# nudro/TFC-GAN

Measured on AMD Instinct MI355X. Metric: training images/sec at 256x256 PATCH-16, 1/2/4/8 MI355X; gen L1 vs ref, higher is better.
Workload: dtype bf16; 1 GPU; PATCH-16 256x256 bf16, batch 32 per GPU (BASELINE.json configs[1]; configs[3] at 8 GPUs): G step + D step, 16-patch triplet + patch-FFT loss, Adam (step as BASELINE.md section 3 defines it: LPIPS and the temperature head excluded); global_batch=32, per_gpu_batch=32, parallelism=dp1

## Files before the change

### tfc-gan_amd/_lib.py

```python
import ctypes
import os
import subprocess
import threading

_HERE = os.path.dirname(os.path.abspath(__file__))
_ROOT = os.path.dirname(_HERE)
CSRC = os.path.join(_HERE, "csrc")
SO_PATH = os.path.join(_HERE, "libtfcgan_hip.so")
SOURCES = ["api.hip", "igemm.hip", "elementwise.hip", "losses.hip", "stn.hip", "lpips.hip", "input.hip", "probe.hip", "vit.hip"]
HEADERS = ["common.h", "tfc_desc.h", "pack_math.h"]
PUBLIC_HEADER = os.path.join(_ROOT, "include", "tfc_gan.h")

DT_BF16, DT_F32 = 0, 1
OP_CONV, OP_PADCONV, OP_CONVT, OP_UPCONV, OP_CONV3 = 0, 1, 2, 3, 4
EP_BIAS, EP_STATS, EP_ACCUM, EP_TANH_NCHW, EP_LEAKY, EP_RELU = 1, 2, 4, 8, 16, 32

_lock = threading.Lock()
_lib = None


def _stale():
    if not os.path.exists(SO_PATH):
        return True
    t = os.path.getmtime(SO_PATH)
    deps = [os.path.join(CSRC, f) for f in SOURCES + HEADERS] + [PUBLIC_HEADER]
    return any(os.path.exists(d) and os.path.getmtime(d) > t for d in deps)


def build(force=False, verbose=False):
    if not force and not _stale():
        return SO_PATH
    import fcntl
    try:
        lk = open(SO_PATH + ".lock", "w")
    except OSError:
        return _build_locked(verbose)
    with lk:
        fcntl.flock(lk, fcntl.LOCK_EX)
        try:
            if not force and not _stale():
                return SO_PATH
            return _build_locked(verbose)
        finally:
            fcntl.flock(lk, fcntl.LOCK_UN)


def _build_locked(verbose):
    hipcc = os.environ.get("HIPCC", "/opt/rocm/bin/hipcc")
    if not os.path.exists(hipcc):
        hipcc = "hipcc"
    cmd = [hipcc, "--offload-arch=gfx950", "-O3", "-std=c++17", "-fPIC", "-shared", "-Wno-unused-value", "-Rpass-analysis=kernel-resource-usage",
           "-Wl,-rpath,/opt/rocm/lib", "-o", SO_PATH + ".tmp"] + [os.path.join(CSRC, f) for f in SOURCES]
    if verbose:
        print(" ".join(cmd))
    res = subprocess.run(cmd, stderr=subprocess.PIPE, text=True)
    if res.returncode != 0:
        raise RuntimeError("hipcc failed:\n" + "\n".join(l for l in res.stderr.splitlines() if "remark:" not in l)[-8000:])
    bad = check_no_spills(res.stderr)
    if bad:
        raise RuntimeError("hand-scheduled kernels must not spill (their asm loads carry hand-counted waits the compiler cannot see): " + "; ".join(bad))
    os.replace(SO_PATH + ".tmp", SO_PATH)
    return SO_PATH


GUARDED_KERNELS = ("tfc_igemm2_kernel", "tfc_wgrad")


def check_no_spills(remarks):
    bad, name = [], None
    for line in remarks.splitlines():
        if "Function Name:" in line:
            name = line.split("Function Name:")[1].split("[")[0].strip()
        elif name and any(g in name for g in GUARDED_KERNELS):
            for key in ("ScratchSize [bytes/lane]:", "VGPRs Spill:"):
                if key in line:
                    val = int(line.split(key)[1].split("[")[0].strip())
                    if val != 0:
                        bad.append(f"{name[:80]}: {key} {val}")
    return bad


_c = ctypes
_vp, _i, _f, _ll, _u32, _sz = _c.c_void_p, _c.c_int, _c.c_float, _c.c_longlong, _c.c_uint32, _c.c_size_t

PROTOTYPES = {
    "tfc_last_error": (_c.c_char_p, []),
    "tfc_abi_version": (_i, []),
    "tfc_part_ws_floats": (_sz, []),
    "tfc_conv_packed_bytes": (_sz, [_i, _i, _i, _i, _i]),
    "tfc_conv_pack": (_i, [_vp, _i, _i, _i, _vp, _vp, _vp, _i, _i]),
    "tfc_pack_plan_bytes": (_sz, [_i]),
    "tfc_pack_plan_build": (_i, [_i, _i, _c.POINTER(_i), _c.POINTER(_i), _c.POINTER(_vp), _c.POINTER(_vp), _c.POINTER(_i), _c.POINTER(_i),
                                 _vp, _c.POINTER(_i)]),
    "tfc_conv_pack_planned": (_i, [_vp, _i, _vp, _i, _i]),
    "tfc_conv_fwd": (_i, [_vp, _i, _i, _vp, _i, _i, _i, _i, _i, _i, _vp, _vp, _i, _vp, _vp, _vp, _vp, _i, _vp]),
    "tfc_conv_dgrad_image": (_i, [_vp, _i, _vp, _i, _i, _i, _i, _i, _i, _vp, _vp, _i, _vp]),
    "tfc_upconv_head_fwd": (_i, [_vp, _i, _vp, _i, _i, _i, _i, _i, _i, _vp, _vp, _vp]),
    "tfc_upconv_head_dgrad": (_i, [_vp, _i, _vp, _i, _i, _i, _i, _i, _i, _vp, _vp, _i]),
    "tfc_patchgan_head_fwd": (_i, [_vp, _i, _vp, _i, _i, _i, _i, _i, _vp, _vp, _i]),
    "tfc_conv_dgrad": (_i, [_vp, _i, _i, _vp, _i, _i, _i, _i, _i, _i, _vp, _vp, _i, _vp, _i]),
    "tfc_conv_wgrad_ws_bytes": (_sz, [_i, _i, _i]),
    "tfc_conv_wgrad": (_i, [_vp, _i, _i, _vp, _i, _vp, _i, _i, _i, _i, _i, _i, _vp, _vp, _i]),
    "tfc_act_fwd": (_i, [_vp, _i, _vp, _i, _i, _i, _i, _i, _vp, _i, _f, _i, _f, _u32, _vp, _i, _vp, _vp]),
    "tfc_act_bwd_signs": (_i, [_vp, _i, _vp, _i, _vp, _i, _i, _i, _i, _f, _vp, _vp, _i, _vp]),
    "tfc_act_bwd": (_i, [_vp, _i, _i, _vp, _i, _vp, _i, _i, _i, _i, _i, _vp, _i, _f, _i, _f, _u32, _vp, _vp, _i, _vp]),
    "tfc_dropout_mask": (_i, [_vp, _vp, _ll, _f, _u32]),
    "tfc_pack_nhwc8": (_i, [_vp, _i, _vp, _i, _vp, _i, _vp, _i, _i, _i]),
    "tfc_unpack_nchw": (_i, [_vp, _i, _vp, _i, _i, _i, _vp, _i, _i, _i, _f, _f]),
    "tfc_tanh_bwd_pack": (_i, [_vp, _i, _vp, _vp, _vp, _vp, _i, _i, _i, _i, _vp]),
    "tfc_colsum": (_i, [_vp, _i, _vp, _ll, _i, _i, _vp, _vp]),
    "tfc_cast": (_i, [_vp, _i, _i, _vp, _vp, _ll]),
    "tfc_axpby": (_i, [_vp, _vp, _vp, _vp, _ll, _f, _f]),
    "tfc_spectral_norm_step": (_i, [_vp, _vp, _vp, _vp, _vp, _vp, _i, _i, _i]),
    "tfc_spectral_norm_batched_ws_floats": (_sz, [_i, _c.POINTER(_i), _c.POINTER(_i)]),
    "tfc_spectral_norm_step_batched": (_i, [_vp, _i, _c.POINTER(_vp), _c.POINTER(_vp), _c.POINTER(_vp), _c.POINTER(_vp), _c.POINTER(_vp),
                                            _c.POINTER(_vp), _c.POINTER(_i), _c.POINTER(_i), _vp, _i]),
    "tfc_spectral_norm_bwd": (_i, [_vp, _vp, _vp, _vp, _vp, _vp, _vp, _vp, _i, _i, _i]),
    "tfc_patch16_triplet": (_i, [_vp, _vp, _vp, _c.POINTER(_i), _i, _i, _vp, _vp, _f]),
    "tfc_fft_spectrum": (_i, [_vp, _vp, _ll, _ll, _i, _i, _i, _i, _i, _i, _vp, _vp, _i, _vp]),
    "tfc_fft_spectrum_ws_bytes": (_sz, [_i, _i]),
    "tfc_logmag_mse": (_i, [_vp, _vp, _vp, _i, _i, _vp]),
    "tfc_logmag_mae": (_i, [_vp, _vp, _vp, _i, _i, _vp]),
    "tfc_vectorize_temps": (_i, [_vp, _vp, _ll, _i, _i, _i, _i, _vp, _vp]),
    "tfc_row_triplet": (_i, [_vp, _vp, _vp, _vp, _ll, _i, _f, _vp]),
    "tfc_l1_sum": (_i, [_vp, _vp, _vp, _ll, _f, _vp, _i]),
    "tfc_affine_warp_fwd": (_i, [_vp, _vp, _vp, _vp, _i, _i, _i, _i]),
    "tfc_affine_warp_bwd": (_i, [_vp, _vp, _vp, _vp, _vp, _vp, _i, _i, _i, _i, _vp]),
    "tfc_morph_grad_fwd": (_i, [_vp, _vp, _vp, _vp, _ll, _i, _i]),
    "tfc_morph_grad_bwd": (_i, [_vp, _vp, _vp, _vp, _ll, _i, _i]),
    "tfc_row_triplet_grad": (_i, [_vp, _vp, _vp, _vp, _ll, _i, _f, _f, _vp, _vp]),
    "tfc_first_block_bwd_supported": (_i, [_i, _i, _i]),
    "tfc_first_block_bwd_wgrad": (_i, [_vp, _i, _vp, _i, _vp, _i, _vp, _i, _i, _i, _i, _i, _i, _f, _vp, _vp, _i, _vp, _vp, _vp]),
    "tfc_conv_first_fwd": (_i, [_vp, _i, _vp, _i, _i, _i, _i, _i, _i, _vp, _vp, _i, _vp, _vp, _i, _vp]),
    "tfc_first_block_fwd": (_i, [_vp, _i, _vp, _i, _i, _i, _i, _i, _i, _vp, _vp, _vp, _f, _i, _vp, _i, _vp]),
    "tfc_resize_plan_bytes": (_sz, [_i, _i, _i]),
    "tfc_resize_plan_build": (_i, [_i, _i, _i, _vp]),
    "tfc_pair_resize_ws_bytes": (_sz, [_i, _i, _i]),
    "tfc_pair_resize_normalize": (_i, [_vp, _vp, _ll, _i, _i, _vp, _vp, _vp, _vp, _vp, _vp, _vp, _vp, _vp]),
    "tfc_lpips_input_fwd": (_i, [_vp, _i, _vp, _vp, _vp, _vp, _i, _i, _i, _i, _i]),
    "tfc_lpips_input_bwd": (_i, [_vp, _i, _vp, _vp, _vp, _i, _i, _i, _i, _i, _f, _i]),
    "tfc_maxpool2_fwd": (_i, [_vp, _i, _vp, _vp, _i, _i, _i, _i]),
    "tfc_maxpool2_bwd": (_i, [_vp, _i, _vp, _vp, _vp, _i, _i, _i, _i]),
    "tfc_relu_bwd": (_i, [_vp, _i, _vp, _vp, _vp, _vp, _ll]),
    "tfc_lpips_head": (_i, [_vp, _i, _vp, _vp, _vp, _vp, _vp, _i, _i, _i, _i, _f]),
    "tfc_bce_relativistic": (_i, [_vp, _i, _vp, _vp, _i, _i, _f, _f, _i, _vp, _vp, _vp, _f]),
    "tfc_adam_step": (_i, [_vp, _vp, _vp, _vp, _vp, _ll, _f, _f, _f, _f, _i, _f]),
    "tfc_prof_enable": (_i, [_i]),
    "tfc_prof_collect": (_i, [_i, _c.POINTER(_c.c_double), _c.POINTER(_c.c_double), _c.POINTER(_ll)]),
# ... 42 lines not shown
```

### tfc-gan_amd/csrc/api.hip

```cpp
#include <hip/hip_runtime.h>
#include <math.h>
#include <stdarg.h>
#include <stdio.h>
#include <string.h>
#include <stdlib.h>
#include <string>
#include <vector>
#include "../../include/tfc_gan.h"
#undef TFC_DT_BF16
#undef TFC_DT_F32
#undef TFC_EP_BIAS
#undef TFC_EP_STATS
#undef TFC_EP_ACCUM
#undef TFC_EP_TANH_NCHW
#undef TFC_EP_LEAKY
#undef TFC_EP_RELU
#undef TFC_OP_CONV
#undef TFC_OP_PADCONV
#undef TFC_OP_CONVT
#undef TFC_OP_UPCONV
#undef TFC_OP_CONV3
#include "tfc_desc.h"
#include "pack_math.h"
#define TFC_OP_CONV 0
#define TFC_OP_PADCONV 1
#define TFC_OP_CONVT 2
#define TFC_OP_UPCONV 3
#define TFC_OP_CONV3 4

int tfc_total_substeps(const TfcGather& d, int es);
int tfc_nb32(int nout);
int tfc_nb32_padded(int nout);
size_t tfc_packed_bytes(const TfcGather& d, int es);
hipError_t tfc_launch_pack(int dt, const TfcGather& d, const float* w, const float* scale, void* wp, int Nreal, int Creal, long long sn, long long sc, hipStream_t st);
hipError_t tfc_launch_igemm(int dt, const TfcGather& d, const void* in, const void* wp, void* out, const float* bias, float* stats, float* part_ws, float* out_nchw, const float* oscale, int flags, hipStream_t st);
hipError_t tfc_launch_first_block_fwd(const void* in, int N, int IH, int IW, const void* wp, const float* bias, const float* oscale, float slope, int gform,
                                      void* out, int o_pitch, unsigned char* sign_mask, hipStream_t st);
bool tfc_conv_c8_eligible(const TfcGather& d, int flags);
hipError_t tfc_launch_conv_c8(const TfcGather& d, const void* in, const void* wp, void* out, const float* bias, const float* oscale, int flags,
                              unsigned char* sign_mask, hipStream_t st);
hipError_t tfc_launch_wgrad(int dt, const TfcGather& d, const void* dO, const void* in, float* dwacc, void* slab, int Nn_pad, int Nn_real, int Cw_real, hipStream_t st, TfcWgradFin* fin);
hipError_t tfc_launch_dgrad_rows4(const void* dy, int dy_pitch, int N, int H, int W, const float* w, int Cin, const float* oscale, int NC, float* dx, hipStream_t st);
hipError_t tfc_launch_upconv_head(const void* x, int x_pitch, int N, int H, int W, const float* w, const float* bias, int Cout, float* out, hipStream_t st);
bool tfc_launch_wgrad_phases_fused(int up, const void* x, int N, int IH, int IW, int x_pitch, int Cin_pad, const void* dy, int dy_pitch, int Cout,
                                   int Cin, float* dwacc, void* slab, hipStream_t st, hipError_t* err, TfcWgradFin* fin);
hipError_t tfc_launch_wgrad_finish(float* acc, float* grad, int Nn, int Cw, long long sn, long long sc, int accumulate, hipStream_t st);
hipError_t tfc_launch_pack_planned(int dt, const void* plan_dev, int njobs, int nblocks, hipStream_t st);
hipError_t tfc_launch_act_fwd(int dt, const ActParams& p, const void* x, const float* stats, void* out, float* stats_out, float* part_ws, hipStream_t st);
hipError_t tfc_launch_act_bwd(int dt, int mode, const ActParams& p, const void* dout, const void* x, const float* stats, float* rstats, void* dx, int use_x, int dx_pitch, float* part_ws, hipStream_t st);
hipError_t tfc_launch_act_pool2_bwd_signs(const ActParams& p, const void* dout, const unsigned char* sign_mask, float* rstats, void* dx, int dx_pitch, float* part_ws, hipStream_t st);
hipError_t tfc_launch_colsum(int dt, const void* x, long long rows, int pitch, int C, float* out, float* part_ws, hipStream_t st);
hipError_t tfc_launch_pack_nhwc8(int dt, const float* a, int Ca, const float* b, int Cb, void* out, int N, int HW, hipStream_t st);
hipError_t tfc_launch_unpack_nchw(int dt, const void* in, int pitch, int c0, int C, float* out, int N, int HW, float alpha, float beta, hipStream_t st);
hipError_t tfc_launch_tanh_bwd_pack(int dt, const float* g, const float* y, void* out, float* dbias, float* part_ws, int N, int C, int HW, hipStream_t st);
hipError_t tfc_launch_sn_bwd(const float* G, const float* W, const float* u, const float* v, const float* sigma2, float* dot_ws, float* gout, int R, int K, int accumulate, hipStream_t st);
hipError_t tfc_launch_bce_rel(int dt, const void* a, const void* b, int n, int stride, float t1, float t2, int mode, float* loss, void* da, void* db, float gscale, hipStream_t st);
hipError_t tfc_launch_adam(float* p, const float* g, float* m, float* v, long long n, float lr, float b1, float b2, float eps, float bc1, float bc2_sqrt, float gscale, hipStream_t st);
hipError_t tfc_launch_axpby(float* out, const float* x, const float* y, long long n, float a, float b, hipStream_t st);
hipError_t tfc_launch_dropout_mask(unsigned char* out, long long n, unsigned seed, unsigned thresh24, hipStream_t st);
hipError_t tfc_launch_cast(int dt, int to_f32, const void* x, void* y, long long n, hipStream_t st);
hipError_t tfc_launch_triplet16(const float* fake, const float* real, const int* neg_idx, int N, int C, float margin, float eps, float* loss, float* dfake, float gscale, hipStream_t st);
hipError_t tfc_launch_spectrum(const float* img, long long bs, long long cs, int rs, int C, int S, int wins_x, int wins_per_img, int nwin, float* amp, float* pha, int shift, void* ws, hipStream_t st);
size_t tfc_fft_ws_bytes(int S, int nwin);
hipError_t tfc_launch_l1_sum(const float* a, const float* b, long long n, float scale, float* out, hipStream_t st);
hipError_t tfc_launch_probe(float* out, hipStream_t st);
hipError_t tfc_launch_logmag_mse(const float* a, const float* b, int S, int nwin, float* out, int absolute, hipStream_t st);
hipError_t tfc_launch_vectorize_temps(const float* x, long long bs, int rs, int N, int H, int W, const float* lut, float* out, hipStream_t st);
hipError_t tfc_launch_row_triplet(const float* a, const float* p, const float* ng, long long rows, int W, float margin, float eps,
                                  float* loss, hipStream_t st);
hipError_t tfc_launch_head_fwd(int dt, const void* x, int x_pitch, const float* w, void* y, int y_pitch, int N, int H, int W, int C, hipStream_t st);
hipError_t tfc_launch_affine_warp_fwd(const float* src, const float* theta, float* out, int N, int C, int H, int W, hipStream_t st);
hipError_t tfc_launch_affine_warp_bwd(const float* src, const float* theta, const float* gout, float* dtheta, float* dsrc, float* part_ws, int N, int C, int H, int W, hipStream_t st);
hipError_t tfc_launch_morph_grad_fwd(const float* x, float* out, unsigned char* arg, long long planes, int H, int W, hipStream_t st);
hipError_t tfc_launch_morph_grad_bwd(const float* gout, const unsigned char* arg, float* dx, long long planes, int H, int W, hipStream_t st);
hipError_t tfc_launch_row_triplet_grad(const float* a, const float* p, const float* ng, long long rows, int W, float margin, float eps, float gscale,
                                       float* loss, float* da, hipStream_t st);
hipError_t tfc_launch_vit_gemm(int dt, const TfcVitGemm& g, float* part_ws, hipStream_t st);
hipError_t tfc_launch_vit_ln_fwd(const float* x, const float* g, const float* b, float* y, float* mean, float* rstd, int rows, int D, float eps, hipStream_t st);
hipError_t tfc_launch_vit_ln_bwd(const float* dy, const float* x, const float* mean, const float* rstd, const float* g, const float* dres, float* dx,
                                 float* dgb, int rows, int D, float* part_ws, hipStream_t st);
hipError_t tfc_launch_vit_colsum(const float* v, long long ld, int rows, int L, const float* x_ln, const float* mean, const float* rstd, float* out,
                                 float* part_ws, hipStream_t st);
hipError_t tfc_launch_vit_attn_fwd(int dt, const float* qkv, float* out, float* probs, int N, int T, int H, float scale, hipStream_t st);
hipError_t tfc_launch_vit_attn_bwd(int dt, const float* dout, const float* qkv, const float* probs, float* dqkv, int N, int T, int H, float scale,
                                   hipStream_t st);
hipError_t tfc_launch_vit_tokens_fwd(float* x, const float* cls, const float* pos, int N, int T, int D, hipStream_t st);
struct SnBatch {
  const float* W[4];
  float* u[4]; float* v[4]; float* sigma2[4];
  float* us[4]; float* vs[4];
  float* s[4]; float* t[4];
  int R[4], K[4];
  int n;
};
hipError_t tfc_launch_sn_step_batched(const SnBatch& b, int power_iter, float eps, hipStream_t st);

static thread_local std::string g_err;
static int fail(int code, const char* fmt, ...) {
  char buf[512];
  va_list ap;
  va_start(ap, fmt);
  vsnprintf(buf, sizeof buf, fmt, ap);
  va_end(ap);
  g_err = buf;
  return code;
}
static int hipfail(hipError_t e, const char* where) { return fail(-100 - (int)e, "%s: %s", where, hipGetErrorString(e)); }
#define CHECK_HIP(expr, where) do { hipError_t e_ = (expr); if (e_ != hipSuccess) return hipfail(e_, where); } while (0)
#define REQUIRE(cond, ...) do { if (!(cond)) return fail(-1, __VA_ARGS__); } while (0)

extern "C" const char* tfc_last_error(void) { return g_err.c_str(); }
extern "C" int tfc_abi_version(void) { return 2; }
extern "C" size_t tfc_part_ws_floats(void) { return (size_t)TFC_PART_WS_FLOATS; }

static inline int pad8(int c) { return (c + 7) / 8 * 8; }
static inline int es_of(int dt) { return dt == TFC_DT_BF16 ? 2 : 4; }

namespace {
// ... 233 lines not shown
  REQUIRE(N > 0 && H > 1 && W > 1 && Cin > 0 && Cout > 0, "bad dims N=%d H=%d W=%d Cin=%d Cout=%d", N, H, W, Cin, Cout);
  REQUIRE((long long)N * (2 * H) * (2 * W) * (long long)(pad8(Cin) > pad8(Cout) ? pad8(Cin) : pad8(Cout)) < 2147483647LL,
          "tensor exceeds 2^31 elements");
  const int es = es_of(dt);
  REQUIRE(pad8(Cin) * es <= 64 || (pad8(Cin) * es) % 64 == 0, "Cin=%d: padded channel bytes must be <= 64 or a multiple of 64", Cin);
  REQUIRE(pad8(Cout) * es <= 64 || (pad8(Cout) * es) % 64 == 0, "Cout=%d: padded channel bytes must be <= 64 or a multiple of 64", Cout);
  REQUIRE(op != TFC_OP_CONV3 || ((pad8(Cin) * es) % 64 == 0 && (pad8(Cout) * es) % 64 == 0), "TFC_OP_CONV3 needs channel bytes in multiples of 64 (Cin=%d Cout=%d)", Cin, Cout);
  return 0;
}
static int check_pitch(int dt, int pitch, int cpad, const char* what) {
  const int ue = 16 / es_of(dt);
  REQUIRE(pitch >= cpad && pitch % ue == 0, "%s pitch %d must be >= %d and a multiple of %d", what, pitch, cpad, ue);
  return 0;
}
static int check_dt(int dt) {
  REQUIRE(dt == TFC_DT_BF16 || dt == TFC_DT_F32, "bad dtype %d", dt);
  return 0;
}
static int check_ptr16(const void* p, const char* what) {
  REQUIRE(p != nullptr && (((uintptr_t)p) & 15) == 0, "%s must be a 16-byte aligned device pointer", what);
  return 0;
}

static size_t phase_packed_offset(int dt, int op, int pass, int Cin, int Cout, int ph) {
  size_t off = 0;
  for (int q = 0; q < ph; ++q) {
    TfcGather d;
    if (build_desc(op, pass, q, 1, 16, 16, Cin, Cout, pad8(Cin), pad8(Cout), &d, nullptr)) return 0;
    off += tfc_packed_bytes(d, es_of(dt));
  }
  return off;
}

extern "C" size_t tfc_conv_packed_bytes(int dt, int op, int pass, int Cin, int Cout) {
  if (pass < 0 || pass > 1 || op < 0 || op > 4) return 0;
  return phase_packed_offset(dt, op, pass, Cin, Cout, num_phases(op, pass));
}

extern "C" int tfc_conv_pack(void* stream, int dt, int op, int pass, const float* w, const float* scale, void* packed, int Cin, int Cout) {
  if (int e = check_common(dt, op, 1, 16, 16, Cin, Cout)) return e;
  REQUIRE(pass == 0 || pass == 1, "pass must be 0 (fwd) or 1 (dgrad)");
  if (int e = check_ptr16(packed, "packed")) return e;
  REQUIRE(w != nullptr, "w is null");
  for (int ph = 0; ph < num_phases(op, pass); ++ph) {
    TfcGather d;
    WeightMap wm;
    if (int e = build_desc(op, pass, ph, 1, 16, 16, Cin, Cout, pad8(Cin), pad8(Cout), &d, &wm)) return e;
    CHECK_HIP(tfc_launch_pack(dt, d, w, scale, (char*)packed + phase_packed_offset(dt, op, pass, Cin, Cout, ph), wm.Nreal, wm.Creal, wm.sn, wm.sc, (hipStream_t)stream), "tfc_conv_pack");
  }
  return 0;
}

extern "C" int tfc_first_block_bwd_supported(int dt, int Cin, int Cout);
static double conv_flop(int op, int N, int H, int W, int Cin, int Cout) {
  const double oh = out_hw(op, H), ow = out_hw(op, W);
  const double taps = (op == TFC_OP_CONVT) ? 4.0 : (op == TFC_OP_CONV3 ? 9.0 : 16.0);
  return 2.0 * N * oh * ow * (double)Cin * Cout * taps;
}

extern "C" int tfc_conv_fwd(void* stream, int dt, int op, const void* x, int x_pitch, int N, int H, int W, int Cin, int Cout,
                            const void* packed, void* y, int y_pitch, const float* bias, float* stats, float* out_nchw, const float* oscale, int flags,
                            float* part_ws) {
  if (int e = check_common(dt, op, N, H, W, Cin, Cout)) return e;
  if (int e = check_ptr16(x, "x")) return e;
  if (int e = check_ptr16(packed, "packed")) return e;
  if (int e = check_pitch(dt, x_pitch, pad8(Cin), "x")) return e;
  if (flags & TFC_EP_TANH_NCHW) { REQUIRE(out_nchw != nullptr, "out_nchw is null"); }
  else {
    REQUIRE(y != nullptr, "y is null");
    REQUIRE(y_pitch >= Cout, "y pitch %d < Cout %d", y_pitch, Cout);
    if (dt == TFC_DT_BF16 && Cout >= 8) REQUIRE(y_pitch % 8 == 0 && (((uintptr_t)y) & 15) == 0, "bf16 outputs are stored in 16-byte units: y must be 16-byte aligned with pitch %% 8 == 0");
  }
  if (flags & TFC_EP_BIAS) REQUIRE(bias != nullptr, "bias is null");
  if (flags & TFC_EP_STATS) REQUIRE(stats != nullptr && part_ws != nullptr, "TFC_EP_STATS needs stats and part_ws");
  int nph = num_phases(op, 0);
  const bool fold = (op == TFC_OP_CONVT || op == TFC_OP_UPCONV);
  if (fold) nph = 1;
  ProfScope prof(0, conv_flop(op, N, H, W, Cin, Cout), (hipStream_t)stream, op, 0, N, H, W, Cin, Cout);
  for (int ph = 0; ph < nph; ++ph) {
    TfcGather d;
    if (int e = build_desc(op, 0, ph, N, H, W, Cin, Cout, x_pitch, y_pitch, &d, nullptr)) return e;
    if (fold) { d.ph_n = 4; d.ph_d0 = (op == TFC_OP_CONVT) ? 1 : 0; d.ph_oo = 1; }
    if (int e = check_desc(d, dt)) return e;
    CHECK_HIP(tfc_launch_igemm(dt, d, x, (const char*)packed + phase_packed_offset(dt, op, 0, Cin, Cout, ph), y, bias, stats, part_ws, out_nchw, oscale, flags, (hipStream_t)stream), "tfc_conv_fwd");
  }
  return 0;
}

extern "C" int tfc_conv_first_fwd(void* stream, int dt, const void* x, int x_pitch, int N, int H, int W, int Cin, int Cout, const void* packed, void* y,
                                  int y_pitch, const float* bias, const float* oscale, int flags, uint8_t* sign_mask) {
  REQUIRE(dt == TFC_DT_BF16 && tfc_first_block_bwd_supported(dt, Cin, Cout), "tfc_conv_first_fwd: bf16, Cin <= 8, Cout == 64 (use tfc_conv_fwd otherwise)");
  if (int e = check_common(dt, TFC_OP_CONV, N, H, W, Cin, Cout)) return e;
  if (int e = check_ptr16(x, "x")) return e;
  if (int e = check_ptr16(packed, "packed")) return e;
  if (int e = check_ptr16(y, "y")) return e;
  REQUIRE(x_pitch == 8 && y_pitch >= Cout && y_pitch % 8 == 0, "pitches: x %d (must be 8), y %d", x_pitch, y_pitch);
  REQUIRE((flags & ~(TFC_EP_BIAS | TFC_EP_LEAKY)) == 0 && (!(flags & TFC_EP_BIAS) || bias), "flags: TFC_EP_BIAS (with bias) | TFC_EP_LEAKY only");
  REQUIRE(!sign_mask || (((uintptr_t)sign_mask) & 7) == 0, "sign_mask must be 8-byte aligned");
  TfcGather d;
  if (int e = build_desc(TFC_OP_CONV, 0, 0, N, H, W, Cin, Cout, x_pitch, y_pitch, &d, nullptr)) return e;
  REQUIRE(tfc_conv_c8_eligible(d, flags), "unexpected descriptor");
  ProfScope prof(0, conv_flop(TFC_OP_CONV, N, H, W, Cin, Cout), (hipStream_t)stream, TFC_OP_CONV, 0, N, H, W, Cin, Cout);
  CHECK_HIP(tfc_launch_conv_c8(d, x, packed, y, bias, oscale, flags, sign_mask, (hipStream_t)stream), "tfc_conv_first_fwd");
  return 0;
}

extern "C" int tfc_first_block_fwd(void* stream, int dt, const void* x, int x_pitch, int N, int H, int W, int Cin, int Cout, const void* packed, const float* bias,
                                   const float* oscale, float slope, int act_after_rounding, void* out, int out_pitch, uint8_t* sign_mask) {
  REQUIRE(dt == TFC_DT_BF16 && tfc_first_block_bwd_supported(dt, Cin, Cout), "tfc_first_block_fwd: bf16, Cin <= 8, Cout == 64");
  if (int e = check_common(dt, TFC_OP_CONV, N, H, W, Cin, Cout)) return e;
  if (int e = check_ptr16(x, "x")) return e;
  if (int e = check_ptr16(packed, "packed")) return e;
  REQUIRE(out && (((uintptr_t)out) & 7) == 0 && out_pitch >= 64 && out_pitch % 4 == 0, "out must be 8-byte aligned with pitch >= 64 and a multiple of 4");
  REQUIRE(x_pitch == 8 && H >= 6 && W >= 6, "x pitch %d (must be 8); the reflect padding of the pooling needs a 5 x 5 convolution output at least", x_pitch);
  REQUIRE(!sign_mask || (((uintptr_t)sign_mask) & 7) == 0, "sign_mask must be 8-byte aligned");
  ProfScope prof(0, conv_flop(TFC_OP_CONV, N, H, W, Cin, Cout), (hipStream_t)stream, TFC_OP_CONV, 0, N, H, W, Cin, Cout);
  CHECK_HIP(tfc_launch_first_block_fwd(x, N, H, W, packed, bias, oscale, slope, act_after_rounding, out, out_pitch, sign_mask, (hipStream_t)stream),
            "tfc_first_block_fwd");
  return 0;
}

extern "C" int tfc_conv_dgrad_image(void* stream, int dt, const void* dy, int dy_pitch, int N, int H, int W, int Cin, int Cout, const float* w,
                                   const float* oscale, int nch, float* dx_nchw) {
  REQUIRE(dt == TFC_DT_BF16 && Cout == 64 && Cin >= 1 && nch >= 1 && nch <= 4 && nch <= Cin, "tfc_conv_dgrad_image: bf16, Cout == 64, nch <= min(4, Cin) only");
  REQUIRE(dy && w && dx_nchw && N > 0 && H > 4 && W > 4 && dy_pitch >= 64 && dy_pitch % 8 == 0, "bad args");
  if (int e = check_ptr16(dy, "dy")) return e;
  ProfScope prof(0, 2.0 * N * (H - 1.0) * (W - 1.0) * nch * Cout * 16.0, (hipStream_t)stream, TFC_OP_CONV, 1, N, H, W, nch, Cout);
  CHECK_HIP(tfc_launch_dgrad_rows4(dy, dy_pitch, N, H, W, w, Cin, oscale, nch, dx_nchw, (hipStream_t)stream), "tfc_conv_dgrad_image");
  return 0;
}

hipError_t tfc_launch_dgrad_head(const void* dy, int dy_pitch, int N, int H, int W, const float* w, int Cout, void* dx, int dx_pitch, hipStream_t st);
extern "C" int tfc_upconv_head_dgrad(void* stream, int dt, const void* dy, int dy_pitch, int N, int H, int W, int Cin, int Cout, const float* w, void* dx,
                                     int dx_pitch) {
  REQUIRE(dt == TFC_DT_BF16 && Cin == 128 && Cout >= 1 && Cout <= 8, "tfc_upconv_head_dgrad: bf16, Cin == 128, Cout <= 8 only (use tfc_conv_dgrad(TFC_OP_UPCONV) otherwise)");
  REQUIRE(dy && w && dx && N > 0 && H > 1 && W > 1 && dy_pitch >= 8 && dy_pitch % 8 == 0 && dx_pitch >= 128 && dx_pitch % 8 == 0, "bad args");
  REQUIRE((long long)N * H * W * dx_pitch < 2147483647LL, "tensor exceeds 2^31 elements");
  if (int e = check_ptr16(dy, "dy")) return e;
  if (int e = check_ptr16(dx, "dx")) return e;
  if (int e = check_ptr16(w, "w")) return e;
  ProfScope prof(0, conv_flop(TFC_OP_UPCONV, N, H, W, Cin, Cout), (hipStream_t)stream, TFC_OP_UPCONV, 1, N, H, W, Cin, Cout);
  CHECK_HIP(tfc_launch_dgrad_head(dy, dy_pitch, N, H, W, w, Cout, dx, dx_pitch, (hipStream_t)stream), "tfc_upconv_head_dgrad");
  return 0;
}

extern "C" int tfc_upconv_head_fwd(void* stream, int dt, const void* x, int x_pitch, int N, int H, int W, int Cin, int Cout, const float* w,
                                  const float* bias, float* out_nchw) {
  REQUIRE(dt == TFC_DT_BF16 && Cin == 128 && Cout >= 1 && Cout <= 4, "tfc_upconv_head_fwd: bf16, Cin == 128, Cout <= 4 only (use tfc_conv_fwd(TFC_OP_UPCONV) otherwise)");
  REQUIRE(x && w && out_nchw && N > 0 && H > 1 && W > 1 && x_pitch >= 128 && x_pitch % 8 == 0, "bad args");
  if (int e = check_ptr16(x, "x")) return e;
  if (int e = check_ptr16(w, "w")) return e;
  ProfScope prof(0, conv_flop(TFC_OP_UPCONV, N, H, W, Cin, Cout), (hipStream_t)stream, TFC_OP_UPCONV, 0, N, H, W, Cin, Cout);
  CHECK_HIP(tfc_launch_upconv_head(x, x_pitch, N, H, W, w, bias, Cout, out_nchw, (hipStream_t)stream), "tfc_upconv_head_fwd");
  return 0;
}

extern "C" int tfc_conv_dgrad(void* stream, int dt, int op, const void* dy, int dy_pitch, int N, int H, int W, int Cin, int Cout,
                              const void* packed, void* dx, int dx_pitch, const float* oscale, int flags) {
  if (int e = check_common(dt, op, N, H, W, Cin, Cout)) return e;
  if (int e = check_ptr16(dy, "dy")) return e;
  if (int e = check_ptr16(packed, "packed")) return e;
  if (int e = check_pitch(dt, dy_pitch, pad8(Cout), "dy")) return e;
  REQUIRE(dx != nullptr && dx_pitch >= Cin, "dx null or pitch %d < Cin %d", dx_pitch, Cin);
  if (dt == TFC_DT_BF16 && Cin >= 8) REQUIRE(dx_pitch % 8 == 0 && (((uintptr_t)dx) & 15) == 0, "bf16 outputs are stored in 16-byte units: dx must be 16-byte aligned with pitch %% 8 == 0");
  REQUIRE((flags & ~TFC_EP_ACCUM) == 0, "dgrad supports only TFC_EP_ACCUM");
  TfcGather d;
  if (int e = build_desc(op, 1, 0, N, H, W, Cin, Cout, dy_pitch, dx_pitch, &d, nullptr)) return e;
  if (int e = check_desc(d, dt)) return e;
  ProfScope prof(0, conv_flop(op, N, H, W, Cin, Cout), (hipStream_t)stream, op, 1, N, H, W, Cin, Cout);
  CHECK_HIP(tfc_launch_igemm(dt, d, dy, packed, dx, nullptr, nullptr, nullptr, nullptr, oscale, flags, (hipStream_t)stream), "tfc_conv_dgrad");
  return 0;
}

struct TfcPackJob {
  TfcGather d;
  const float* w;
  void* wp;
  long long sn, sc;
  int NB32, Nreal, Creal, units;
  int first_block, threads;
};
extern "C" size_t tfc_pack_plan_bytes(int nlayers) { return (size_t)nlayers * 4 * sizeof(TfcPackJob); }
extern "C" int tfc_pack_plan_build(int dt, int nlayers, const int* ops, const int* passes, const float* const* w, void* const* packed,
                                   const int* Cin, const int* Cout, void* plan_host, int* nblocks) {
  REQUIRE(nlayers > 0 && ops && passes && w && packed && Cin && Cout && plan_host && nblocks, "bad args");
  TfcPackJob* jobs = (TfcPackJob*)plan_host;
  int nj = 0, blk = 0;
  for (int l = 0; l < nlayers; ++l) {
    if (int e = check_common(dt, ops[l], 1, 16, 16, Cin[l], Cout[l])) return e;
    REQUIRE(passes[l] == 0 || passes[l] == 1, "pass must be 0 or 1");
    for (int ph = 0; ph < num_phases(ops[l], passes[l]); ++ph) {
      TfcPackJob& j = jobs[nj];
      WeightMap wm;
      if (int e = build_desc(ops[l], passes[l], ph, 1, 16, 16, Cin[l], Cout[l], pad8(Cin[l]), pad8(Cout[l]), &j.d, &wm)) return e;
      j.w = w[l];
      j.wp = (char*)packed[l] + phase_packed_offset(dt, ops[l], passes[l], Cin[l], Cout[l], ph);
      j.sn = wm.sn; j.sc = wm.sc; j.Nreal = wm.Nreal; j.Creal = wm.Creal;
      j.NB32 = tfc_nb32_padded(j.d.Nout);
      j.units = tfc_total_substeps(j.d, es_of(dt)) * j.NB32 * 64;
      j.threads = j.NB32 * 32 * ((j.d.Cin_pad * es_of(dt)) / 16);
      j.first_block = blk;
      blk += (j.threads + 255) / 256;
      ++nj;
    }
  }
  *nblocks = blk;
  return nj;
}
extern "C" int tfc_conv_pack_planned(void* stream, int dt, const void* plan_dev, int njobs, int nblocks) {
  REQUIRE(plan_dev && njobs > 0 && nblocks > 0, "bad args");
  CHECK_HIP(tfc_launch_pack_planned(dt, plan_dev, njobs, nblocks, (hipStream_t)stream), "tfc_conv_pack_planned");
  return 0;
}

extern "C" int tfc_patchgan_head_fwd(void* stream, int dt, const void* x, int x_pitch, int N, int H, int W, int C, const float* w,
                                     void* y, int y_pitch) {
  REQUIRE(dt == TFC_DT_BF16 || dt == TFC_DT_F32, "bad dtype");
  if (int e = check_ptr16(x, "x")) return e;
  const int ue = 16 / es_of(dt);
  REQUIRE(w && y && N > 0 && H > 0 && W > 0 && C > 0 && C % ue == 0 && C <= 2048 && x_pitch >= C && x_pitch % ue == 0 && y_pitch >= 1, "bad args");
  CHECK_HIP(tfc_launch_head_fwd(dt, x, x_pitch, w, y, y_pitch, N, H, W, C, (hipStream_t)stream), "tfc_patchgan_head_fwd");
  return 0;
}

static size_t wgrad_acc_bytes(int Cin, int Cout) { return (((size_t)16 * Cin * Cout * sizeof(float)) + 255) & ~(size_t)255; }
static const size_t kWgradSlabBytes = (size_t)512 * 4 * 8 * 4 * 64 * 16;
extern "C" size_t tfc_conv_wgrad_ws_bytes(int op, int Cin, int Cout) { (void)op; return wgrad_acc_bytes(Cin, Cout) + kWgradSlabBytes; }

extern "C" int tfc_conv_wgrad(void* stream, int dt, int op, const void* x, int x_pitch, const void* dy, int dy_pitch, int N, int H, int W,
                              int Cin, int Cout, void* ws, float* dw, int accumulate) {
  if (int e = check_common(dt, op, N, H, W, Cin, Cout)) return e;
  if (int e = check_ptr16(x, "x")) return e;
  if (int e = check_ptr16(dy, "dy")) return e;
  if (int e = check_pitch(dt, x_pitch, pad8(Cin), "x")) return e;
  if (int e = check_pitch(dt, dy_pitch, pad8(Cout), "dy")) return e;
  REQUIRE(ws != nullptr && dw != nullptr, "ws / dw null");
  REQUIRE(op != TFC_OP_CONV3, "TFC_OP_CONV3 (frozen VGG features of the LPIPS term) has no weight-gradient pass");
  hipStream_t st = (hipStream_t)stream;
  WeightMap wm{};
  TfcWgradFin fin{dw, 0, 0, accumulate, false};
  {
    ProfScope prof(1, conv_flop(op, N, H, W, Cin, Cout), st, op, 2, N, H, W, Cin, Cout);
    bool fused = false;
    if ((op == TFC_OP_CONVT || op == TFC_OP_UPCONV) && dt == TFC_DT_BF16) {
      TfcGather d0;
      if (int e = build_desc(op, 2, 0, N, H, W, Cin, Cout, x_pitch, dy_pitch, &d0, &wm)) return e;
      fin.sn = wm.sn; fin.sc = wm.sc;
      hipError_t herr = hipSuccess;
      fused = tfc_launch_wgrad_phases_fused(op == TFC_OP_UPCONV, x, N, H, W, x_pitch, pad8(Cin), dy, dy_pitch, Cout, Cin,
                                            (float*)((char*)ws + kWgradSlabBytes), ws, st, &herr, &fin);
      if (fused) CHECK_HIP(herr, "tfc_conv_wgrad (phase-fused)");
    }
    const int nph = num_phases(op, 2);
// ... 576 lines not shown
```

Measured before the change: 3569 images/sec.

## Add split-K MFMA kernel for small-spatial-plane convolutions in forward and dgrad

New measurement: 3588 images/sec (median of 5 runs). No clear change (+0.5%).

```diff
diff --git a/tfc-gan_amd/_lib.py b/tfc-gan_amd/_lib.py
--- a/tfc-gan_amd/_lib.py
+++ b/tfc-gan_amd/_lib.py
@@ -7,7 +7,7 @@
 _ROOT = os.path.dirname(_HERE)
 CSRC = os.path.join(_HERE, "csrc")
 SO_PATH = os.path.join(_HERE, "libtfcgan_hip.so")
-SOURCES = ["api.hip", "igemm.hip", "elementwise.hip", "losses.hip", "stn.hip", "lpips.hip", "input.hip", "probe.hip", "vit.hip"]
+SOURCES = ["api.hip", "igemm.hip", "elementwise.hip", "losses.hip", "stn.hip", "lpips.hip", "input.hip", "probe.hip", "vit.hip", "smallplane.hip"]
 HEADERS = ["common.h", "tfc_desc.h", "pack_math.h"]
 PUBLIC_HEADER = os.path.join(_ROOT, "include", "tfc_gan.h")
 
@@ -63,7 +63,7 @@
     return SO_PATH
 
 
-GUARDED_KERNELS = ("tfc_igemm2_kernel", "tfc_wgrad")
+GUARDED_KERNELS = ("tfc_igemm2_kernel", "tfc_wgrad", "tfc_smallplane")
 
 
 def check_no_spills(remarks):
diff --git a/tfc-gan_amd/csrc/api.hip b/tfc-gan_amd/csrc/api.hip
--- a/tfc-gan_amd/csrc/api.hip
+++ b/tfc-gan_amd/csrc/api.hip
@@ -34,6 +34,9 @@
 size_t tfc_packed_bytes(const TfcGather& d, int es);
 hipError_t tfc_launch_pack(int dt, const TfcGather& d, const float* w, const float* scale, void* wp, int Nreal, int Creal, long long sn, long long sc, hipStream_t st);
 hipError_t tfc_launch_igemm(int dt, const TfcGather& d, const void* in, const void* wp, void* out, const float* bias, float* stats, float* part_ws, float* out_nchw, const float* oscale, int flags, hipStream_t st);
+bool tfc_smallplane_eligible(const TfcGather& d, int flags);
+hipError_t tfc_launch_smallplane(const TfcGather& d, const void* in, const void* wp, void* out, const float* bias, float* stats, float* part_ws,
+                                 const float* oscale, int flags, hipStream_t st);
 hipError_t tfc_launch_first_block_fwd(const void* in, int N, int IH, int IW, const void* wp, const float* bias, const float* oscale, float slope, int gform,
                                       void* out, int o_pitch, unsigned char* sign_mask, hipStream_t st);
 bool tfc_conv_c8_eligible(const TfcGather& d, int flags);
@@ -433,7 +436,11 @@
     if (int e = build_desc(op, 0, ph, N, H, W, Cin, Cout, x_pitch, y_pitch, &d, nullptr)) return e;
     if (fold) { d.ph_n = 4; d.ph_d0 = (op == TFC_OP_CONVT) ? 1 : 0; d.ph_oo = 1; }
     if (int e = check_desc(d, dt)) return e;
-    CHECK_HIP(tfc_launch_igemm(dt, d, x, (const char*)packed + phase_packed_offset(dt, op, 0, Cin, Cout, ph), y, bias, stats, part_ws, out_nchw, oscale, flags, (hipStream_t)stream), "tfc_conv_fwd");
+    const void* wp = (const char*)packed + phase_packed_offset(dt, op, 0, Cin, Cout, ph);
+    if (dt == TFC_DT_BF16 && op != TFC_OP_CONV3 && tfc_smallplane_eligible(d, flags))
+      CHECK_HIP(tfc_launch_smallplane(d, x, wp, y, bias, stats, part_ws, oscale, flags, (hipStream_t)stream), "tfc_conv_fwd");
+    else
+      CHECK_HIP(tfc_launch_igemm(dt, d, x, wp, y, bias, stats, part_ws, out_nchw, oscale, flags, (hipStream_t)stream), "tfc_conv_fwd");
   }
   return 0;
 }
@@ -519,7 +526,10 @@
   if (int e = build_desc(op, 1, 0, N, H, W, Cin, Cout, dy_pitch, dx_pitch, &d, nullptr)) return e;
   if (int e = check_desc(d, dt)) return e;
   ProfScope prof(0, conv_flop(op, N, H, W, Cin, Cout), (hipStream_t)stream, op, 1, N, H, W, Cin, Cout);
-  CHECK_HIP(tfc_launch_igemm(dt, d, dy, packed, dx, nullptr, nullptr, nullptr, nullptr, oscale, flags, (hipStream_t)stream), "tfc_conv_dgrad");
+  if (dt == TFC_DT_BF16 && op != TFC_OP_CONV3 && tfc_smallplane_eligible(d, flags))
+    CHECK_HIP(tfc_launch_smallplane(d, dy, packed, dx, nullptr, nullptr, nullptr, oscale, flags, (hipStream_t)stream), "tfc_conv_dgrad");
+  else
+    CHECK_HIP(tfc_launch_igemm(dt, d, dy, packed, dx, nullptr, nullptr, nullptr, nullptr, oscale, flags, (hipStream_t)stream), "tfc_conv_dgrad");
   return 0;
 }
 
diff --git a/tfc-gan_amd/csrc/smallplane.hip b/tfc-gan_amd/csrc/smallplane.hip
--- /dev/null
+++ b/tfc-gan_amd/csrc/smallplane.hip
@@ -0,0 +1,216 @@
+#include <cstdlib>
+#include "common.h"
+
+size_t tfc_packed_bytes(const TfcGather& d, int es);
+int tfc_nb32_padded(int nout);
+
+#define TFC_SP_NT 2
+#define TFC_SP_D 4
+
+template <int MT>
+__global__ void __launch_bounds__(256, 2)
+tfc_smallplane_kernel(const TfcGather d, const bf16_t* __restrict__ in, const unsigned char* __restrict__ wp, bf16_t* out,
+                      const float* __restrict__ bias, float* part, const float* __restrict__ oscale, int flags, int NB32,
+                      long long phase_wbytes, int mtiles, int nslots, int quarter) {
+  constexpr int NT = TFC_SP_NT, D = TFC_SP_D, TM = 32 * MT, NF = MT * NT;
+  extern __shared__ __attribute__((aligned(16))) float red[];
+  const int tid = threadIdx.x, lane = tid & 63;
+  const int wave = __builtin_amdgcn_readfirstlane(tid >> 6);
+  const int r = lane & 31, h = lane >> 5;
+
+  const int nph = d.ph_n > 1 ? d.ph_n : 1;
+  const int item = tfc_xcd_remap(blockIdx.x, gridDim.x);
+  const int nb = item / (mtiles * nph);
+  const int rest = item - nb * mtiles * nph;
+  const int phase = rest / mtiles, mt = rest - phase * mtiles;
+  const int phy = phase >> 1, phx = phase & 1;
+  const int P = d.GH * d.GW, M = d.nimg * P;
+
+  int ibase[MT], ay[MT], bx[MT];
+  bool mok[MT];
+#pragma unroll
+  for (int mi = 0; mi < MT; ++mi) {
+    const int m = mt * TM + mi * 32 + r;
+    mok[mi] = m < M;
+    const int mm = mok[mi] ? m : 0;
+    const int img = mm / P, pix = mm - img * P;
+    const int a = pix / d.GW, b = pix - a * d.GW;
+    ibase[mi] = img * d.IH * d.IW;
+    ay[mi] = a + phy * d.ph_d0;
+    bx[mi] = b + phx * d.ph_d0;
+  }
+
+  const int SPL = 2 * d.plane[0].ntaps;
+  const int PCH = d.nplanes * SPL;
+  const unsigned char* wb = wp + (size_t)phase * (size_t)phase_wbytes + (size_t)(nb * NT) * 1024 + (size_t)lane * 16;
+  const size_t wstep = (size_t)NB32 * 1024;
+
+  u32x4_t ra[D][MT], rb[D][NT];
+  unsigned okm[D];
+  auto load = [&](int i, u32x4_t (&a)[MT], u32x4_t (&b)[NT], unsigned& ok) {
+    const int ii = i < quarter ? i : quarter - 1;
+    const int gs = (((ii >> 1) << 2) + wave) * 2 + (ii & 1);
+    const int cc = gs / PCH, q = gs - cc * PCH;
+    const int pl = q / SPL, s = q - pl * SPL;
+    const TfcPlane& pd = d.plane[pl];
+    const int t = s >> 1;
+    const int oy = pd.dy0 + pd.tap_dy[t], ox = pd.dx0 + pd.tap_dx[t];
+    const int coff = cc * 32 + (2 * (s & 1) + h) * 8;
+    ok = 0;
+#pragma unroll
+    for (int mi = 0; mi < MT; ++mi) {
+      const int Y = (ay[mi] + oy) * d.SS + pd.py, X = (bx[mi] + ox) * d.SS + pd.px;
+      const bool v = mok[mi] && (unsigned)Y < (unsigned)d.IH && (unsigned)X < (unsigned)d.IW;
+      const bf16_t* src = v ? in + (size_t)(ibase[mi] + Y * d.IW + X) * d.in_pitch + coff : in;
+      a[mi] = *reinterpret_cast<const u32x4_t*>(src);
+      ok |= v ? (1u << mi) : 0u;
+    }
+    const unsigned char* pw = wb + (size_t)gs * wstep;
+#pragma unroll
+    for (int nt = 0; nt < NT; ++nt) b[nt] = *reinterpret_cast<const u32x4_t*>(pw + nt * 1024);
+  };
+
+  f32x16_t acc[MT][NT];
+#pragma unroll
+  for (int mi = 0; mi < MT; ++mi)
+#pragma unroll
+    for (int nt = 0; nt < NT; ++nt)
+#pragma unroll
+      for (int j = 0; j < 16; ++j) acc[mi][nt][j] = 0.f;
+
+#pragma unroll
+  for (int j = 0; j < D; ++j) load(j, ra[j], rb[j], okm[j]);
+  for (int i = 0; i < quarter; i += D) {
+#pragma unroll
+    for (int j = 0; j < D; ++j) {
+      const u32x4_t z = {0u, 0u, 0u, 0u};
+#pragma unroll
+      for (int mi = 0; mi < MT; ++mi) {
+        const u32x4_t av = (okm[j] >> mi) & 1u ? ra[j][mi] : z;
+#pragma unroll
+        for (int nt = 0; nt < NT; ++nt)
+          acc[mi][nt] = __builtin_amdgcn_mfma_f32_32x32x16_bf16(__builtin_bit_cast(bf16x8_t, av), __builtin_bit_cast(bf16x8_t, rb[j][nt]),
+                                                                acc[mi][nt], 0, 0, 0);
+      }
+      load(i + j + D, ra[j], rb[j], okm[j]);
+    }
+  }
+
+#pragma unroll
+  for (int mi = 0; mi < MT; ++mi)
+#pragma unroll
+    for (int nt = 0; nt < NT; ++nt)
+#pragma unroll
+      for (int j = 0; j < 16; ++j) red[((wave * NF + mi * NT + nt) * 16 + j) * 64 + lane] = acc[mi][nt][j];
+  __syncthreads();
+  const float osc = oscale ? *oscale : 1.f;
+  float vout[16];
+  int fo = -1;
+  if (wave < NF) {
+    fo = wave;
+    const int n = nb * 64 + (fo % NT) * 32 + r;
+    const float bv = (flags & TFC_EP_BIAS) ? bias[n] : 0.f;
+#pragma unroll
+    for (int j = 0; j < 16; ++j) {
+      float s = red[((0 * NF + fo) * 16 + j) * 64 + lane];
+#pragma unroll
+      for (int w = 1; w < 4; ++w) s += red[((w * NF + fo) * 16 + j) * 64 + lane];
+      float v = s * osc + bv;
+      if (flags & TFC_EP_LEAKY) v = fmaxf(v, 0.2f * v);
+      if (flags & TFC_EP_RELU) v = fmaxf(v, 0.f);
+      vout[j] = bf16_to_f32(f32_to_bf16(v));
+    }
+  }
+  __syncthreads();
+  if (fo >= 0) {
+    const int mi = fo / NT, nt = fo % NT;
+    const int n = nb * 64 + nt * 32 + r;
+#pragma unroll
+    for (int j = 0; j < 16; ++j) {
+      const int row = mi * 32 + (j & 3) + 8 * (j >> 2) + 4 * h;
+      const int m = mt * TM + row;
+      float v = vout[j];
+      if (m < M) {
+        const int img = m / P, pix = m - img * P;
+        const int a = pix / d.GW, b = pix - a * d.GW;
+        const int oy = a * d.OS + d.OOY + phy * d.ph_oo, ox = b * d.OS + d.OOX + phx * d.ph_oo;
+        bf16_t* po = out + ((size_t)(img * d.OH + oy) * d.OW + ox) * d.out_pitch + n;
+        if (flags & TFC_EP_ACCUM) v = bf16_to_f32(f32_to_bf16(v + bf16_to_f32(*po)));
+        *po = f32_to_bf16(v);
+      }
+      if (flags & TFC_EP_STATS) red[row * 64 + nt * 32 + r] = v;
+    }
+  }
+  if (flags & TFC_EP_STATS) {
+    __syncthreads();
+    if (tid < 64) {
+      const int n = nb * 64 + tid;
+      const int nparts = nph * nslots;
+      float2* pp = reinterpret_cast<float2*>(part);
+      int cur = -1;
+      float s1 = 0.f, s2 = 0.f;
+      auto flush = [&]() {
+        const int j = mt - (cur * P) / TM;
+        pp[((size_t)cur * nparts + phase * nslots + j) * d.Nout + n] = make_float2(s1, s2);
+        if ((cur * P + P - 1) / TM == mt)
+          for (int jj = j + 1; jj < nslots; ++jj) pp[((size_t)cur * nparts + phase * nslots + jj) * d.Nout + n] = make_float2(0.f, 0.f);
+      };
+      for (int row = 0; row < TM; ++row) {
+        const int m = mt * TM + row;
+        if (m >= M) break;
+        const int img = m / P;
+        if (img != cur) {
+          if (cur >= 0) flush();
+          cur = img; s1 = 0.f; s2 = 0.f;
+        }
+        const float v = red[row * 64 + tid];
+        s1 += v; s2 += v * v;
+      }
+      if (cur >= 0) flush();
+    }
+  }
+}
+
+bool tfc_smallplane_eligible(const TfcGather& d, int flags) {
+  static const bool off = [] { const char* e = getenv("TFC_NO_SMALL_PLANES"); return e && atoi(e) != 0; }();
+  if (off || g_tfc_force_cfg >= 0) return false;
+  if (flags & TFC_EP_TANH_NCHW) return false;
+  if (d.GH * d.GW > (TFC_TILE_H * TFC_TILE_W) / 4) return false;
+  if ((d.Cin_pad * 2) % 64 != 0 || d.Nout % 64 != 0 || d.out_pitch % 8 != 0) return false;
+  if (d.nplanes != 1 && d.nplanes != 4) return false;
+  for (int pl = 1; pl < d.nplanes; ++pl)
+    if (d.plane[pl].ntaps != d.plane[0].ntaps) return false;
+  const int total = (d.Cin_pad / 32) * d.nplanes * 2 * d.plane[0].ntaps;
+  return total % (8 * TFC_SP_D) == 0;
+}
+
+hipError_t tfc_launch_part_reduce(const float* part, float* out, int G, int nparts, int L, hipStream_t st);
+
+hipError_t tfc_launch_smallplane(const TfcGather& d, const void* in, const void* wp, void* out, const float* bias, float* stats, float* part_ws,
+                                 const float* oscale, int flags, hipStream_t st) {
+  const int nph = d.ph_n > 1 ? d.ph_n : 1;
+  const int M = d.nimg * d.GH * d.GW;
+  const int nblk = d.Nout / 64;
+  const int total = (d.Cin_pad / 32) * d.nplanes * 2 * d.plane[0].ntaps;
+  const int quarter = total / 4;
+  const long long phase_wbytes = (long long)tfc_packed_bytes(d, 2);
+  const int mt64 = (M + 63) / 64;
+  const int MT = (mt64 * nph * nblk >= 256) ? 2 : 1;
+  const int TM = 32 * MT;
+  const int mtiles = (M + TM - 1) / TM;
+  const int P = d.GH * d.GW;
+  const int nslots = (P + TM - 1) / TM + 1;
+  if (flags & TFC_EP_STATS) {
+    if (!stats || !part_ws || (long long)d.nimg * nph * nslots * d.Nout * 2 > (long long)TFC_PART_WS_FLOATS) return hipErrorInvalidValue;
+  }
+  const dim3 grid(mtiles * nph * nblk);
+  const size_t lds = (size_t)4 * MT * TFC_SP_NT * 16 * 64 * 4;
+  if (MT == 2)
+    TFC_LAUNCH(tfc_smallplane_kernel<2>, grid, dim3(256), lds, st, d, (const bf16_t*)in, (const unsigned char*)wp, (bf16_t*)out, bias, part_ws,
+               oscale, flags, tfc_nb32_padded(d.Nout), phase_wbytes, mtiles, nslots, quarter);
+  else
+    TFC_LAUNCH(tfc_smallplane_kernel<1>, grid, dim3(256), lds, st, d, (const bf16_t*)in, (const unsigned char*)wp, (bf16_t*)out, bias, part_ws,
+               oscale, flags, tfc_nb32_padded(d.Nout), phase_wbytes, mtiles, nslots, quarter);
+  if (flags & TFC_EP_STATS) return tfc_launch_part_reduce(part_ws, stats, d.nimg, nph * nslots, 2 * d.Nout, st);
+  return hipGetLastError();
+}
```
